# raviraj988/3D-POINT-CLOUD-SEGMENTATION-USING-2D-IMG-SEGMENTATION

Measured on AMD Instinct MI355X. Metric: labelled points/sec (10M pts x 64 views) at 1/2/4/8 GPU; % HBM roofline, higher is better.
Workload: dtype f64; 1 GPU; C3: 10000000 points x 64 ring views, 1024x1024 block64 uint8 masks, nclasses=133, threshold=0.5, filter_classes=None; fused project->sample->vote->segment; points_total=10000000, points_per_gpu=10000000, views=64, xyz_storage=f64, cloud_layout=caller order, cell-sorted inside every step (F3D_FUSE_SORT), exchange=none

## Files before the change

### 3d-point-cloud-segmentation-using-2d-img-segmentation_amd/csrc/f3d_fuse.hip

```cpp
#include <hip/hip_runtime.h>
#include <stdint.h>
#include <stdlib.h>
#include <string.h>
#include "f3d.h"
#include "f3d_math.h"
#include "f3d_kernels.h"
#include <cstdlib>

#pragma clang fp contract(off)

#define F3D_NO_PREFILL ((int64_t)0x7fffffffffffffffLL)
#define F3D_PART_MAX_GROUPS 16
#ifndef F3D_MID_DENSE
#define F3D_MID_DENSE 8
#endif
#ifndef F3D_NT_CLASSES
#define F3D_NT_CLASSES 1
#endif
#if defined(F3D_EXP_STORE) && F3D_EXP_STORE == 2
#define F3D_STORE_CLASS(p, v) ((void)(v))
#elif defined(F3D_EXP_STORE) && F3D_EXP_STORE == 3
#define F3D_STORE_CLASS(p, v) (reinterpret_cast<uint8_t*>(classes)[(p) - classes] = (uint8_t)(v))
#elif defined(F3D_EXP_STORE) && F3D_EXP_STORE == 4
#define F3D_STORE_CLASS(p, v) __builtin_nontemporal_store((uint8_t)(v), reinterpret_cast<uint8_t*>(classes) + ((p) - classes))
// ... 320 lines not shown
    bool bad = false;
};

template <int MODE>
__device__ __forceinline__ void vote_add(vote_state<MODE>& st, uint32_t* hist, int tid, const f3d_filter_args& flt, int nclasses,
                                         bool valid, int label) {
    using HT = hist_traits<MODE>;
    st.bad = st.bad | (valid & (label > nclasses));
    valid = valid & (label <= nclasses);
    st.total += valid ? 1 : 0;
    const unsigned l = valid ? (unsigned)label : (unsigned)nclasses + 1u;
    const unsigned sh = (l & (HT::per_word - 1)) * HT::bits;
    const uint32_t old = atomicAdd(&hist[(l >> HT::shift) * F3D_BLOCK + tid], 1u << sh);
    const unsigned c = ((old >> sh) & HT::mask) + 1u;
    const unsigned key = valid ? ((c << 16) | (0xFFFFu - l)) : 0u;
    st.best = st.best > key ? st.best : key;
}

template <typename FilterAt>
__device__ __forceinline__ int64_t segment_point(int win_c, int win_i, int total, int nfilter, FilterAt fat, int nclasses, double threshold,
                                                 const uint16_t* cmin = nullptr) {
    int64_t cls;
    if (total == 0) cls = nclasses;
    else {
        cls = win_i;
        const bool low = cmin ? win_c < (int)cmin[total] : (double)win_c / (double)total < threshold;
        if (low) cls = nclasses;
        if (win_c == 0) cls = nclasses;
    }
    if (nfilter > 0) {
        int64_t r = cls;
        for (int k = 0; k < nfilter; ++k) if (r == k) r = fat(k);
        cls = r;
    }
    return cls;
}

template <int MODE, bool WRITE_VOTES>
__device__ __forceinline__ void finish_point(const vote_state<MODE>& st, const uint32_t* hist, int tid, const f3d_filter_args& flt,
                                             int nclasses, double threshold, bool store, int64_t orig,
                                             int64_t* __restrict__ classes, uint16_t* __restrict__ votes_out) {
    using HT = hist_traits<MODE>;
    const int ncols = nclasses + 1;
    int win_c, win_i;
    if (flt.nfilter > 0) {
        win_c = -1; win_i = 0;
        for (int k = 0; k < flt.nfilter; ++k) {
            const int l = f3d_filter_at(flt, k);
            int c = 0;
            if (l >= 0 && l < ncols) c = (int)((hist[(l >> HT::shift) * F3D_BLOCK + tid] >> ((l & (HT::per_word - 1)) * HT::bits)) & HT::mask);
            if (c > win_c) { win_c = c; win_i = k; }
        }
    } else {
        win_c = (int)(st.best >> 16); win_i = (int)(0xFFFFu - (st.best & 0xFFFFu));
    }
    const int64_t cls = segment_point(win_c, win_i, st.total, flt.nfilter, [&](int k) { return f3d_filter_at(flt, k); }, nclasses, threshold);
    if (store) F3D_STORE_CLASS(&classes[orig], cls);
    if (WRITE_VOTES && store) {
        for (int l = 0; l < ncols; ++l)
            votes_out[(size_t)orig * ncols + l] =
                (uint16_t)((hist[(l >> HT::shift) * F3D_BLOCK + tid] >> ((l & (HT::per_word - 1)) * HT::bits)) & HT::mask);
    }
}

__device__ __forceinline__ void vote_bin32(uint32_t* hcol, unsigned b) { atomicAdd(&hcol[b * F3D_BLOCK], 1u); }

template <bool WRITE_VOTES>
__device__ __forceinline__ void finish_bin32(const uint32_t* hcol, int ncodes, const uint8_t* lut, const uint8_t* inv, int nfilter,
                                             const int* __restrict__ fcls, int nclasses, double threshold, bool store, int orig,
                                             int64_t* __restrict__ classes, uint16_t* __restrict__ votes_out, bool& bad,
                                             const uint16_t* cmin = nullptr, int64_t prefilled = F3D_NO_PREFILL) {
    const int ncols = nclasses + 1;
    const unsigned cbad = hcol[F3D_BLOCK];
    bad = cbad != 0u;
    unsigned best = 0, sum = cbad;
    for (int c = 2; c < ncodes; ++c) {
        const unsigned n = hcol[c * F3D_BLOCK];
        const unsigned key = (n << 8) | (unsigned)c;
        sum += n;
        best = best > key ? best : key;
    }
    int win_c, win_i;
    if (nfilter > 0) {
        win_c = -1; win_i = 0;
        for (int k = 0; k < nfilter; ++k) {
            const int l = fcls[k];
            int c = 0;
            if (l >= 0 && l < ncols) { const unsigned b = lut[l]; c = b >= 2u ? (int)hcol[b * F3D_BLOCK] : 0; }
            if (c > win_c) { win_c = c; win_i = k; }
        }
    } else {
        win_c = (int)(best >> 8); win_i = (int)inv[best & 0xFFu];
    }
    const int64_t cls = segment_point(win_c, win_i, (int)sum, nfilter, [&](int k) { return fcls[k]; }, nclasses, threshold, cmin);
    if (store && cls != prefilled) F3D_STORE_CLASS(&classes[orig], cls);
    if (WRITE_VOTES && store) {
        for (int l = 0; l < ncols; ++l) { const unsigned b = lut[l]; votes_out[(size_t)orig * ncols + l] = (uint16_t)(b >= 2u ? hcol[b * F3D_BLOCK] : 0u); }
    }
}

template <bool GUARD>
__device__ __forceinline__ void vote_coded(unsigned& nvalid, uint32_t* hcol, unsigned b) {
    if (GUARD) {
        const unsigned one = b < 1u ? b : 1u;
        nvalid += one;
        atomicAdd(&hcol[(b >> 2) * F3D_BLOCK], one << ((b & 3u) * 8u));
    } else {
        atomicAdd(&hcol[(b >> 2) * F3D_BLOCK], 1u << ((b & 3u) * 8u));
    }
}

__device__ __forceinline__ unsigned coded_count(const uint32_t* hcol, unsigned b) {
    return (hcol[(b >> 2) * F3D_BLOCK] >> ((b & 3u) * 8u)) & 0xFFu;
}

template <bool WRITE_VOTES, bool WRAP>
__device__ __forceinline__ bool finish_coded(unsigned nvalid, const uint32_t* hcol, int words, const uint8_t* lut, const uint8_t* inv,
                                             int nfilter, const int* __restrict__ fcls, int nclasses, double threshold, bool store,
                                             int orig, int64_t* __restrict__ classes, uint16_t* __restrict__ votes_out, bool& bad,
                                             const uint16_t* cmin = nullptr, int64_t prefilled = F3D_NO_PREFILL) {
    const int ncols = nclasses + 1;
    unsigned best = 0, sum = 0;
    {
        const unsigned x = hcol[0];
        bad = ((x >> 8) & 0xFFu) != 0u;
        const unsigned c2 = (x >> 16) & 0xFFu, c3 = x >> 24;
        sum = ((x >> 8) & 0xFFu) + c2 + c3;
        best = (c2 << 8) | 2u;
        const unsigned k3 = (c3 << 8) | 3u;
        best = best > k3 ? best : k3;
    }
    typedef unsigned short u16x2 __attribute__((ext_vector_type(2)));
    u16x2 me = {0, 0}, mo = {0, 0};
    for (int w = 1; w < words; ++w) {
        const unsigned x = hcol[w * F3D_BLOCK];
        const unsigned tag = (unsigned)w * 0x00010001u;
        sum = __builtin_amdgcn_sad_u8(x, 0u, sum);
        const unsigned o = (x & 0xFF00FF00u) | tag, e = ((x << 8) & 0xFF00FF00u) | tag;
        mo = __builtin_elementwise_max(mo, __builtin_bit_cast(u16x2, o));
        me = __builtin_elementwise_max(me, __builtin_bit_cast(u16x2, e));
    }
    {
        const unsigned cand[4] = {me.x, mo.x, me.y, mo.y};
#pragma unroll
        for (unsigned j = 0; j < 4; ++j) {
            const unsigned key = (cand[j] & 0xFF00u) | ((cand[j] & 0x3Fu) << 2) | j;
            best = best > key ? best : key;
        }
    }
    if (WRAP && sum != nvalid) return false;
    int win_c, win_i;
    if (nfilter > 0) {
        win_c = -1; win_i = 0;
        for (int k = 0; k < nfilter; ++k) {
            const int l = fcls[k];
            int c = 0;
            if (l >= 0 && l < ncols) { const unsigned b = lut[l]; c = b >= 2u ? (int)coded_count(hcol, b) : 0; }
            if (c > win_c) { win_c = c; win_i = k; }
        }
    } else {
        win_c = (int)(best >> 8); win_i = (int)inv[best & 0xFFu];
    }
    const int64_t cls = segment_point(win_c, win_i, (int)sum, nfilter, [&](int k) { return fcls[k]; }, nclasses, threshold, cmin);
    if (store && cls != prefilled) F3D_STORE_CLASS(&classes[orig], cls);
    if (WRITE_VOTES && store) {
        for (int l = 0; l < ncols; ++l) { const unsigned b = lut[l]; votes_out[(size_t)orig * ncols + l] = (uint16_t)(b >= 2u ? coded_count(hcol, b) : 0u); }
    }
    return true;
}

template <bool MAX>
__device__ __forceinline__ float wave_reduce(float v) {
#define F3D_DPP_CHAIN(op)                                                                  \
    asm volatile("s_nop 1\n\t" op " %0, %0, %0 quad_perm:[1,0,3,2] row_mask:0xf bank_mask:0xf\n\t" \
                 "s_nop 1\n\t" op " %0, %0, %0 quad_perm:[2,3,0,1] row_mask:0xf bank_mask:0xf\n\t" \
                 "s_nop 1\n\t" op " %0, %0, %0 row_half_mirror row_mask:0xf bank_mask:0xf\n\t"     \
                 "s_nop 1\n\t" op " %0, %0, %0 row_mirror row_mask:0xf bank_mask:0xf\n\t"          \
                 "s_nop 1\n\t" op " %0, %0, %0 row_bcast:15 row_mask:0xa bank_mask:0xf\n\t"        \
                 "s_nop 1\n\t" op " %0, %0, %0 row_bcast:31 row_mask:0xc bank_mask:0xf\n\t"        \
                 "s_nop 1" : "+v"(v))
    if (MAX) F3D_DPP_CHAIN("v_max_f32_dpp"); else F3D_DPP_CHAIN("v_min_f32_dpp");
#undef F3D_DPP_CHAIN
    return __int_as_float(__builtin_amdgcn_readlane(__float_as_int(v), 63));
}

__device__ __forceinline__ void wave_box(float& lo0, float& hi0, float& lo1, float& hi1, float& lo2, float& hi2) {
#define F3D_STEP(ctrl)                                                \
    "v_min_f32_dpp %0, %0, %0 " ctrl "\n\tv_max_f32_dpp %1, %1, %1 " ctrl "\n\t" \
    "v_min_f32_dpp %2, %2, %2 " ctrl "\n\tv_max_f32_dpp %3, %3, %3 " ctrl "\n\t" \
    "v_min_f32_dpp %4, %4, %4 " ctrl "\n\tv_max_f32_dpp %5, %5, %5 " ctrl "\n\t"
    asm volatile("s_nop 1\n\t"
                 F3D_STEP("quad_perm:[1,0,3,2] row_mask:0xf bank_mask:0xf")
                 F3D_STEP("quad_perm:[2,3,0,1] row_mask:0xf bank_mask:0xf")
                 F3D_STEP("row_half_mirror row_mask:0xf bank_mask:0xf")
                 F3D_STEP("row_mirror row_mask:0xf bank_mask:0xf")
                 F3D_STEP("row_bcast:15 row_mask:0xa bank_mask:0xf")
                 F3D_STEP("row_bcast:31 row_mask:0xc bank_mask:0xf")
                 "s_nop 1"
                 : "+v"(lo0), "+v"(hi0), "+v"(lo1), "+v"(hi1), "+v"(lo2), "+v"(hi2));
#undef F3D_STEP
#define F3D_L63(x) x = __int_as_float(__builtin_amdgcn_readlane(__float_as_int(x), 63))
    F3D_L63(lo0); F3D_L63(hi0); F3D_L63(lo1); F3D_L63(hi1); F3D_L63(lo2); F3D_L63(hi2);
#undef F3D_L63
}

#ifndef F3D_VTAB_GLOBAL
#define F3D_VTAB_GLOBAL 0
#endif
#ifndef F3D_XCD_CHUNK_LOG2
#define F3D_XCD_CHUNK_LOG2 6
#endif
#ifndef F3D_FUSE_WAVES
#define F3D_FUSE_WAVES 3
#endif
__device__ __forceinline__ void threshold_table(f3d_codebook* __restrict__ cb, double threshold);
__global__ __launch_bounds__(F3D_BLOCK) void k_fuse_setup(const f3d_view* __restrict__ views, int nviews, float* __restrict__ ctabT,
                                                           double* __restrict__ vtabT, f3d_codebook* __restrict__ cb, double threshold,
                                                           unsigned int* __restrict__ todo_count, int lut_nclasses, int lut_book, f3d_filter_args flt) {
    if (lut_book >= 0 && blockIdx.x == gridDim.x - 1) { code_lut_block(cb, lut_nclasses, lut_book, flt); return; }
    if (blockIdx.x == 0) {
        threshold_table(cb, threshold);
        if (todo_count && threadIdx.x < 4) todo_count[threadIdx.x] = 0u;
    }
    const int ngroups = (nviews + 63) >> 6;
    const int nsetup = lut_book >= 0 ? (int)gridDim.x - 1 : (int)gridDim.x;
    for (int k = blockIdx.x * F3D_BLOCK + threadIdx.x; k < ngroups * 64 * 39; k += nsetup * F3D_BLOCK) {
        const int v = k / 39, f = k - v * 39, g = v >> 6, l = v & 63;
        const f3d_view& vw = views[v < nviews ? v : nviews - 1];
        if (f < 24) ctabT[(g * 24 + f) * 64 + l] = reinterpret_cast<const float*>(&vw.cull_n32[0][0])[f];
        else vtabT[(g * F3D_VHEAD + (f - 24)) * 64 + l] = reinterpret_cast<const double*>(&vw)[f - 24];
    }
}

template <typename T, int PPL, bool WRITE_VOTES, bool BIN32, bool WRAP, bool TLDS, bool CARRY>
__global__ __launch_bounds__(F3D_BLOCK, F3D_FUSE_WAVES) void k_fuse(const T* __restrict__ xyz, int64_t n,
                                                     const f3d_view* __restrict__ views, int nviews,
                                                     const uint8_t* __restrict__ cmasks, int H, int W,
                                                     int nclasses, int nfilter, const int* __restrict__ fcls, double threshold,
                                                     int64_t* __restrict__ classes, uint16_t* __restrict__ votes_out,
                                                     int* __restrict__ err, const int32_t* __restrict__ perm, int gather_xyz,
                                                     unsigned int* __restrict__ todo_count, int32_t* __restrict__ todo,
                                                     const f3d_codebook* __restrict__ cb, int cmin, int cmax,
                                                     const float* __restrict__ ctabT, const double* __restrict__ vtabT,
                                                     uint32_t* __restrict__ carry, int chunk_flags, T* __restrict__ xyz_keep,
                                                     unsigned long long* __restrict__ umask, uint32_t* __restrict__ park, int park_slots, int park_stride,
                                                     int64_t prefilled) {
    const int ncodes = cb->ncodes;
    if (ncodes > cmax || ncodes < cmin) return;
    const int words = (ncodes + 3) >> 2;
    const int hdw = BIN32 ? ncodes : words;
    extern __shared__ uint32_t lds_u32[];
    float* ctab = reinterpret_cast<float*>(lds_u32);
    uint32_t* lutw = TLDS ? lds_u32 + 64 * F3D_CULL_ROW : lds_u32;
    double* vtab = reinterpret_cast<double*>(lutw + F3D_BOOK_DWORDS);
    uint32_t* hist = (TLDS && !F3D_VTAB_GLOBAL) ? lutw + F3D_BOOK_DWORDS + 2 * F3D_VHEAD * 64 : lutw + F3D_BOOK_DWORDS;
    const uint16_t* vmin = (WRAP || nviews > 255) ? nullptr : reinterpret_cast<const uint16_t*>(lutw + 128);
    const uint8_t* lut = reinterpret_cast<const uint8_t*>(lutw);
    const uint8_t* inv = lut + 256;
    const int tid = threadIdx.x, lane = threadIdx.x & 63;
    constexpr int TILE = F3D_BLOCK * PPL;
    const int npts = (int)n;
    const int ntiles = (int)((n + TILE - 1) / TILE);
    const unsigned plane = (unsigned)f3d_coded_plane(H, W);
    const int pitch = f3d_coded_pitch(W);
    const int c_row = 64 * pitch - 64;
    const int ngroups = (nviews + 63) >> 6;
    const float umaxf = (float)(W > H ? W : H), Wf = (float)W, Hf = (float)H;

    const __amdgpu_buffer_rsrc_t cm_rsrc = __builtin_amdgcn_make_buffer_rsrc(const_cast<uint8_t*>(cmasks), 0, (int)((unsigned)nviews * plane), 0x00020000);
#if defined(F3D_EXP_GATHER) && F3D_EXP_GATHER == 1
    auto gather = [&](unsigned off) -> unsigned { return (unsigned)__builtin_amdgcn_raw_buffer_load_b8(cm_rsrc, (int)(off & 63u), 0, 0); };
#elif defined(F3D_EXP_GATHER) && F3D_EXP_GATHER == 2
    auto gather = [&](unsigned off) -> unsigned { return off & 2u; };
#else
    auto gather = [&](unsigned off) -> unsigned { return (unsigned)__builtin_amdgcn_raw_buffer_load_b8(cm_rsrc, (int)off, 0, 0); };
#endif
    lutw[tid] = reinterpret_cast<const uint32_t*>(cb->lut)[tid];
    auto stage_group = [&](int g) {
        const int nv = min(64, nviews - 64 * g);
        for (int k = tid; k < nv * 24; k += F3D_BLOCK) {
            const int vi = k / 24, f = k - vi * 24;
            ctab[vi * F3D_CULL_ROW + f] = reinterpret_cast<const float*>(&views[64 * g + vi].cull_n32[0][0])[f];
        }
        if (!F3D_VTAB_GLOBAL)
            for (int k = tid; k < nv * F3D_VHEAD; k += F3D_BLOCK) {
                const int vi = k / F3D_VHEAD, f = k - vi * F3D_VHEAD;
                vtab[f * 64 + vi] = reinterpret_cast<const double*>(&views[64 * g + vi])[f];
            }
    };
    if (TLDS && ngroups > 1) return;
    if (TLDS) stage_group(0);
    __syncthreads();

    int xlog = F3D_XCD_CHUNK_LOG2;
#ifndef F3D_XCD_MIN_ROWS
#define F3D_XCD_MIN_ROWS 8
#endif
    while (xlog > 0 && ntiles < ((8 * F3D_XCD_MIN_ROWS) << xlog)) --xlog;
    const int chunk_rows = (ntiles + (8 << xlog) - 1) >> (xlog + 3);
    const int tiles_per_xcd = chunk_rows << xlog;
    const int xcd = blockIdx.x & 7, bx = blockIdx.x >> 3, gx = gridDim.x >> 3;
    uint32_t* const hcol0 = hist + tid;
    uint32_t* const hcol1 = PPL == 2 ? hist + hdw * F3D_BLOCK + tid : hcol0;
    for (int j = bx; j < tiles_per_xcd; j += gx) {
        const int tile = ((j >> xlog) << (xlog + 3)) + (xcd << xlog) + (j & ((1 << xlog) - 1));
        if (tile >= ntiles) continue;
        const int i0 = tile * TILE + (tid >> 6) * (64 * PPL) + lane;
        bool live[2], act[2], defer[2];
        int orig[2];
        f32x2 DX, DY, DZ;
        float c0, c1, c2, e0, e1, e2, ps_box;
        bool wave_any;
        {
            f3d_p3 p[2];
            float lo0 = INFINITY, lo1 = INFINITY, lo2 = INFINITY, hi0 = -INFINITY, hi1 = -INFINITY, hi2 = -INFINITY;
#pragma unroll
            for (int q = 0; q < 2; ++q) {
                const int i = i0 + 64 * q;
                live[q] = (q < PPL) & (i < npts);
                orig[q] = live[q] ? (perm ? perm[i] : i) : i;
                p[q].x = p[q].y = p[q].z = 0.0;
                if (live[q]) p[q] = f3d_load_p3(xyz, (int64_t)(gather_xyz ? orig[q] : i));
                if (CARRY && xyz_keep && live[q]) { xyz_keep[3 * (size_t)i] = (T)p[q].x; xyz_keep[3 * (size_t)i + 1] = (T)p[q].y; xyz_keep[3 * (size_t)i + 2] = (T)p[q].z; }
                const double pscale = (fabs(p[q].x) + fabs(p[q].y)) + fabs(p[q].z);
                act[q] = live[q] & (pscale < 1.0e30);
                defer[q] = live[q] & !act[q];
                const float x32 = (float)p[q].x, y32 = (float)p[q].y, z32 = (float)p[q].z;
                if (act[q]) {
                    lo0 = fminf(lo0, x32); hi0 = fmaxf(hi0, x32); lo1 = fminf(lo1, y32); hi1 = fmaxf(hi1, y32);
                    lo2 = fminf(lo2, z32); hi2 = fmaxf(hi2, z32);
                }
            }
            wave_box(lo0, hi0, lo1, hi1, lo2, hi2);
            wave_any = __any(act[0] | act[1]);
            c0 = 0.5f * (lo0 + hi0); c1 = 0.5f * (lo1 + hi1); c2 = 0.5f * (lo2 + hi2);
            e0 = 0.5f * (hi0 - lo0) * 1.000002f + 1e-30f; e1 = 0.5f * (hi1 - lo1) * 1.000002f + 1e-30f;
            e2 = 0.5f * (hi2 - lo2) * 1.000002f + 1e-30f;
            ps_box = ((fabsf(c0) + fabsf(c1)) + fabsf(c2)) + ((e0 + e1) + e2);
            DX = (f32x2){(float)(p[0].x - (double)c0), (float)(p[1].x - (double)c0)};
            DY = (f32x2){(float)(p[0].y - (double)c1), (float)(p[1].y - (double)c1)};
            DZ = (f32x2){(float)(p[0].z - (double)c2), (float)(p[1].z - (double)c2)};
            if (!act[0]) { DX.x = __builtin_nanf(""); }
            if (!act[1]) { DX.y = __builtin_nanf(""); }
        }
        constexpr bool PART = !CARRY;
        const bool part_rt = PART && park_slots > 0 && ngroups <= F3D_PART_MAX_GROUPS;
        unsigned long long um[2] = {0ull, 0ull};
        int slot[2] = {-1, -1};
        unsigned unsure[2] = {0u, 0u};
        if (CARRY && (chunk_flags & 1)) {
#pragma unroll
            for (int q = 0; q < PPL; ++q) {
                uint32_t* hc = q ? hcol1 : hcol0;
                const uint32_t* cq = carry + ((size_t)(tile * PPL + q) * words) * F3D_BLOCK + tid;
                for (int wd = 0; wd < words; ++wd) {
                    uint32_t x = cq[wd * F3D_BLOCK];
                    if (wd == 0) { defer[q] = defer[q] | (live[q] & ((x & 0xFFu) != 0u)); x &= ~0xFFu; }
                    if (BIN32) {
#pragma unroll
                        for (int b4 = 0; b4 < 4; ++b4) if (4 * wd + b4 < ncodes) hc[(4 * wd + b4) * F3D_BLOCK] = (x >> (8 * b4)) & 0xFFu;
                    } else {
                        hc[wd * F3D_BLOCK] = x;
                    }
                }
            }
        } else {
            for (int wd = 0; wd < hdw; ++wd) { hcol0[wd * F3D_BLOCK] = 0u; if (PPL == 2) hcol1[wd * F3D_BLOCK] = 0u; }
        }
        unsigned nvalid[2] = {0u, 0u};
        unsigned pend[2] = {F3D_CODE_NONE, F3D_CODE_NONE};
        unsigned ccode[2][F3D_CHUNK];
#pragma unroll
        for (int k = 0; k < F3D_CHUNK; ++k) ccode[0][k] = ccode[1][k] = F3D_CODE_NONE;
#if F3D_GATHER_DEPTH == 2
        unsigned ccode2[2][F3D_CHUNK];
#pragma unroll
        for (int k = 0; k < F3D_CHUNK; ++k) ccode2[0][k] = ccode2[1][k] = F3D_CODE_NONE;
#define F3D_OLDEST ccode2
#else
#define F3D_OLDEST ccode
#endif
        auto vote = [&](int q, unsigned b) {
            if (q >= PPL) return;
            if (BIN32) vote_bin32(q ? hcol1 : hcol0, b);
            else vote_coded<WRAP || CARRY>(nvalid[q], q ? hcol1 : hcol0, b);
        };

        for (int g = 0; g < ngroups; ++g) {
            const int vj = 64 * g + lane;
            bool box_out = false, box_in = true, own_image = false;
            float pb0 = 0.f, pb1 = 0.f, pb2 = 0.f, pb3 = 0.f, pb4 = 0.f, pmarg = 0.f;
            unsigned pneed = 0u;
            if (vj < nviews) {
                const float* rowp = TLDS ? ctab + lane * F3D_CULL_ROW : ctabT + (size_t)g * 24 * 64 + lane;
                auto rowf = [&](int f) { return TLDS ? rowp[f] : rowp[f * 64]; };
                const float marg = 2.0f * __builtin_fmaf(rowf(20), ps_box, rowf(21));
                float bmax = 0.f, smax = 0.f, base[F3D_NPLANES];
                unsigned need = 0u;
#pragma unroll
                for (int m = 0; m < F3D_NPLANES; ++m) {
                    const float n0 = rowf(3 * m), n1 = rowf(3 * m + 1), n2 = rowf(3 * m + 2);
                    base[m] = __builtin_fmaf(n0, c0, __builtin_fmaf(n1, c1, __builtin_fmaf(n2, c2, -rowf(15 + m))));
                    const float spread = __builtin_fmaf(fabsf(n0), e0, __builtin_fmaf(fabsf(n1), e1, fabsf(n2) * e2));
                    box_out = box_out | (base[m] + spread < -marg);
                    box_in = box_in & (base[m] - spread > marg);
                    need |= (base[m] - spread > marg) ? 0u : (1u << m);
                    bmax = fmaxf(bmax, fabsf(base[m])); smax = fmaxf(smax, spread);
                }
                pb0 = base[0]; pb1 = base[1]; pb2 = base[2]; pb3 = base[3]; pb4 = base[4];
                pneed = need;
                pmarg = 0.5f * marg + 1.01f * (float)F3D_U24 * (4.0f * bmax + 5.0f * smax);
                own_image = (int)(rowf(22) == Wf) & (int)(rowf(23) == Hf);
            }
            centre_row mine = {0.f, 0.f, 0.f, 0.f, 0.f, 0.f, 0.f, 0.f, 0.f, 0.f, 0.f, 0.f, 0u, 0, 0};
            bool row_ok = false;
            if (vj < nviews && !box_out && wave_any)
                row_ok = centre_precompute((TLDS && !F3D_VTAB_GLOBAL) ? vtab + lane : vtabT + (size_t)g * F3D_VHEAD * 64 + lane, 64, c0, c1, c2, e0, e1, e2, umaxf, pitch, mine);
            mine.obase += (unsigned)vj * plane;
            const unsigned long long valid_m = __ballot(vj < nviews);
            unsigned long long out_m = __ballot(vj < nviews && box_out);
            const unsigned long long in_m = __ballot(vj < nviews && box_in && !box_out && own_image);
            const unsigned long long row_m = __ballot(row_ok);
            if (!wave_any) out_m = valid_m;
            unsigned long long todo_v = valid_m & ~out_m & in_m & row_m;
#if defined(F3D_EXP_SKIP) && (F3D_EXP_SKIP == 1 || F3D_EXP_SKIP == 3)
            todo_v = 0ull;
#endif
            while (todo_v) {
                int cbit[F3D_CHUNK]; unsigned coff[2][F3D_CHUNK];
                bool use[F3D_CHUNK];
                unsigned long long unsm[2][F3D_CHUNK];
#pragma unroll
                for (int k = 0; k < F3D_CHUNK; ++k) {
                    use[k] = todo_v != 0ull;
                    cbit[k] = use[k] ? __builtin_ctzll(todo_v) : (k ? cbit[0] : 0);
                    if (use[k]) todo_v &= todo_v - 1ull;
                }
#pragma unroll
                for (int k = 0; k < F3D_CHUNK; ++k) {
                    const centre_row r = read_row(mine, cbit[k]);
                    int fi0[2], fi1[2]; bool safe[2];
                    project_offset2(r, DX, DY, DZ, fi0, fi1, safe);
#pragma unroll
                    for (int q = 0; q < PPL; ++q) {
                        if (PART) unsm[q][k] = __ballot(act[q] & !safe[q]);
                        else unsure[q] = safe[q] ? unsure[q] : 1u;
                        const unsigned o = r.obase + rel_offset(fi0[q], fi1[q], c_row);
                        coff[q][k] = (safe[q] & use[k]) ? o : 0u;
                    }
                }
#ifndef F3D_NO_VOTE_PIN
#pragma unroll
                for (int k = 0; k < F3D_CHUNK; ++k) {
                    asm volatile("" : "+v"(F3D_OLDEST[0][k]) : "v"(coff[0][k]));
                    if (PPL == 2) asm volatile("" : "+v"(F3D_OLDEST[1][k]) : "v"(coff[1][k]));
                }
#endif
#pragma unroll
                for (int k = 0; k < F3D_CHUNK; ++k) { vote(0, F3D_OLDEST[0][k]); vote(1, F3D_OLDEST[1][k]); }
#if F3D_GATHER_DEPTH == 2
#pragma unroll
                for (int k = 0; k < F3D_CHUNK; ++k) { ccode2[0][k] = ccode[0][k]; ccode2[1][k] = ccode[1][k]; }
#endif
#pragma unroll
                for (int k = 0; k < F3D_CHUNK; ++k) { ccode[0][k] = gather(coff[0][k]); if (PPL == 2) ccode[1][k] = gather(coff[1][k]); }
                if (PART) {
                    unsigned long long au = 0ull;
#pragma unroll
                    for (int k = 0; k < F3D_CHUNK; ++k) au |= unsm[0][k] | (PPL == 2 ? unsm[1][k] : 0ull);
                    if (__builtin_expect(au != 0ull, 0)) {
                        asm volatile("" ::: "memory");
                        const unsigned long long me = 1ull << lane;
#pragma unroll
                        for (int k = 0; k < F3D_CHUNK; ++k)
#pragma unroll
                            for (int q = 0; q < PPL; ++q) um[q] |= (unsm[q][k] & me) ? (1ull << cbit[k]) : 0ull;
                    }
                }
            }
#pragma unroll
            for (int k = 0; k < F3D_CHUNK; ++k) {
#if F3D_GATHER_DEPTH == 2
                vote(0, ccode2[0][k]); vote(1, ccode2[1][k]);
                ccode2[0][k] = ccode2[1][k] = F3D_CODE_NONE;
#endif
                vote(0, ccode[0][k]); vote(1, ccode[1][k]);
                ccode[0][k] = ccode[1][k] = F3D_CODE_NONE;
            }
            todo_v = valid_m & ~out_m & ~(in_m & row_m);
#if defined(F3D_EXP_SKIP) && F3D_EXP_SKIP == 2
            todo_v = 0ull;
#elif defined(F3D_EXP_SKIP) && F3D_EXP_SKIP == 3
            todo_v = 0ull;
#endif
            while (todo_v) {
                const int bit = __builtin_ctzll(todo_v);
                todo_v &= todo_v - 1ull;
                const int v = 64 * g + bit;
                const f3d_view& vw = views[v];
                float nn[F3D_NPLANES][3];
#pragma unroll
                for (int m = 0; m < F3D_NPLANES; ++m) { nn[m][0] = vw.cull_n32[m][0]; nn[m][1] = vw.cull_n32[m][1]; nn[m][2] = vw.cull_n32[m][2]; }
#pragma unroll
                for (int m = 0; m < F3D_NPLANES; ++m) { asm volatile("" : "+s"(nn[m][0])); asm volatile("" : "+s"(nn[m][1])); asm volatile("" : "+s"(nn[m][2])); }
#define F3D_RL1(x) __int_as_float(__builtin_amdgcn_readlane(__float_as_int(x), bit))
                const float mg = F3D_RL1(pmarg);
                const unsigned need = (unsigned)__builtin_amdgcn_readlane((int)pneed, bit);
                const float* pbs[F3D_NPLANES] = {&pb0, &pb1, &pb2, &pb3, &pb4};
                const bool has_row = (row_m >> bit) & 1ull;
                bool maybe[2] = {true, true}, sure[2] = {true, true};
#pragma unroll
                for (int m = 0; m < F3D_NPLANES; ++m) {
                    if (!((need >> m) & 1u)) continue;
                    const float bbm = F3D_RL1(*pbs[m]);
                    const f32x2 a = F3D_FMA2(splat2(nn[m][0]), DX, F3D_FMA2(splat2(nn[m][1]), DY, F3D_FMA2(splat2(nn[m][2]), DZ, splat2(bbm))));
                    maybe[0] = maybe[0] & (a.x > -mg); sure[0] = sure[0] & (a.x > mg);
                    maybe[1] = maybe[1] & (a.y > -mg); sure[1] = sure[1] & (a.y > mg);
                }
#undef F3D_RL1
                unsigned off[2] = {0u, 0u};
                bool unsv[2] = {false, false};
                if (has_row) {
                    centre_row r = read_row(mine, bit);
                    const int U8 = __builtin_amdgcn_readlane(mine.U8, bit), V8 = __builtin_amdgcn_readlane(mine.V8, bit);
                    int fi0[2], fi1[2]; bool safe[2];
                    project_offset2(r, DX, DY, DZ, fi0, fi1, safe);
#pragma unroll
                    for (int q = 0; q < PPL; ++q) {
                        const bool inside = sure[q];
                        const bool hit = inside & safe[q] & ((unsigned)(fi0[q] + U8) < (unsigned)W) & ((unsigned)(fi1[q] + V8) < (unsigned)H);
                        unsv[q] = (maybe[q] & !sure[q]) | (inside & !safe[q]);
                        const unsigned o = r.obase + rel_offset(fi0[q], fi1[q], c_row);
                        off[q] = hit ? o : 0u;
                    }
                } else {
#pragma unroll
                    for (int q = 0; q < PPL; ++q) unsv[q] = maybe[q];
                }
                if (PART) {
                    const unsigned long long u0 = __ballot(unsv[0] & act[0]), u1 = __ballot(unsv[1] & act[1]);
                    if (__builtin_expect((u0 | u1) != 0ull, 0)) {
                        asm volatile("" ::: "memory");
                        const unsigned long long me = 1ull << lane;
                        um[0] |= (u0 & me) ? (1ull << bit) : 0ull;
                        if (PPL == 2) um[1] |= (u1 & me) ? (1ull << bit) : 0ull;
                    }
                } else {
#pragma unroll
                    for (int q = 0; q < PPL; ++q) unsure[q] = unsv[q] ? 1u : unsure[q];
                }
#ifndef F3D_NO_VOTE_PIN
                asm volatile("" : "+v"(pend[0]) : "v"(off[0]));
                if (PPL == 2) asm volatile("" : "+v"(pend[1]) : "v"(off[1]));
#endif
                vote(0, pend[0]); vote(1, pend[1]);
                pend[0] = gather(off[0]); if (PPL == 2) pend[1] = gather(off[1]);
            }
            if (PART && __any(((um[0] | um[1]) != 0ull) | (slot[0] >= 0) | (slot[1] >= 0))) {
#pragma unroll
                for (int q = 0; q < PPL; ++q) {
                    if (!part_rt) { unsure[q] = um[q] != 0ull ? 1u : unsure[q]; }
                    else if (act[q] && (um[q] != 0ull || slot[q] >= 0)) {
                        if (slot[q] < 0) {
                            slot[q] = (int)atomicAdd(todo_count, 1u);
                            if (slot[q] < park_slots) for (int gg = 0; gg < g; ++gg) umask[(size_t)slot[q] * ngroups + gg] = 0ull;
                        }
                        if (slot[q] < park_slots) umask[(size_t)slot[q] * ngroups + g] = um[q];
                    }
                    um[q] = 0ull;
                }
            }
        }
#pragma unroll
        for (int q = 0; q < PPL; ++q) {
            vote(q, pend[q]);
            const bool part = act[q] & ((PART && slot[q] >= 0) | (unsure[q] != 0u));
            bool full = defer[q] | (part & !part_rt);
            defer[q] = defer[q] | part;
            uint32_t* hc = q ? hcol1 : hcol0;
            if (CARRY && (chunk_flags & 2)) {
                uint32_t* cq = carry + ((size_t)(tile * PPL + q) * words) * F3D_BLOCK + tid;
                for (int wd = 0; wd < words; ++wd) {
                    uint32_t x = 0u;
                    if (BIN32) {
#pragma unroll
                        for (int b4 = 0; b4 < 4; ++b4) if (4 * wd + b4 < ncodes) x |= (hc[(4 * wd + b4) * F3D_BLOCK] & 0xFFu) << (8 * b4);
                    } else {
                        x = hc[wd * F3D_BLOCK];
                    }
                    if (wd == 0) x = (x & ~0xFFu) | (defer[q] ? 1u : 0u);
                    cq[wd * F3D_BLOCK] = x;
                }
                continue;
            }
            bool bad = false, trusted = true;
            if (BIN32) finish_bin32<WRITE_VOTES>(hc, ncodes, lut, inv, nfilter, fcls, nclasses, threshold, live[q] & !defer[q], orig[q], classes, votes_out, bad, vmin, prefilled);
            else trusted = finish_coded<WRITE_VOTES, WRAP>(nvalid[q], hc, words, lut, inv, nfilter, fcls, nclasses, threshold, live[q] & !defer[q], orig[q],
                                                           classes, votes_out, bad, vmin, prefilled);
            full = full | (live[q] & !trusted);
            const bool d = defer[q] | full;
            if (d) {
                const int sl = (PART && slot[q] >= 0) ? slot[q] : (int)atomicAdd(todo_count, 1u);
                full = full | !part_rt | (sl >= park_slots) | !(PART && slot[q] >= 0);
                if (BIN32 && !full && nviews > 255)
                    for (int c = 1; c < ncodes; ++c) full = full | (hc[c * F3D_BLOCK] > 255u);
                todo[sl] = (gather_xyz ? orig[q] : (i0 + 64 * q)) | (full ? (int)0x80000000 : 0);
                if (PART && !full) {
                    uint32_t* pk = park + (size_t)sl * park_stride;
                    for (int wd = 0; wd < words; ++wd) {
                        uint32_t x = 0u;
                        if (BIN32) {
#pragma unroll
                            for (int b4 = 0; b4 < 4; ++b4) if (4 * wd + b4 < ncodes) x |= (hc[(4 * wd + b4) * F3D_BLOCK] & 0xFFu) << (8 * b4);
                        } else {
                            x = hc[wd * F3D_BLOCK];
                        }
                        pk[wd] = wd == 0 ? (x & ~0xFFu) : x;
                    }
                }
            }
            if (bad & !d) atomicOr(err, F3D_DEVERR_FUSE);
        }
    }
}

__device__ __forceinline__ void cull_point64(const f3d_view& vw, f3d_p3 p, double pscale, bool& maybe, bool& sure) {
    const double marg = __builtin_fma(vw.cull_rel64, pscale, vw.cull_abs64);
    bool mb = true, sr = true;
#pragma unroll
    for (int m = 0; m < F3D_NPLANES; ++m) {
        const double a = __builtin_fma(vw.plane_n[m][0], p.x, __builtin_fma(vw.plane_n[m][1], p.y,
                         __builtin_fma(vw.plane_n[m][2], p.z, -vw.plane_off[m])));
        mb = mb & (a > -marg);
        sr = sr & (a > marg);
    }
    maybe = mb; sure = sr;
}

__device__ __forceinline__ bool project_fast(const f3d_view& vw, double umax, f3d_p3 p, int W, int H, int& iu, int& iv, bool& unsure) {
    const double d0 = p.x - vw.t[0], d1 = p.y - vw.t[1], d2 = p.z - vw.t[2];
    const double h0 = __builtin_fma(vw.M[0], d0, __builtin_fma(vw.M[1], d1, vw.M[2] * d2));
    const double h1 = __builtin_fma(vw.M[3], d0, __builtin_fma(vw.M[4], d1, vw.M[5] * d2));
    const double h2 = __builtin_fma(vw.M[6], d0, __builtin_fma(vw.M[7], d1, vw.M[8] * d2));
    const double r = rcp_newton(h2);
    const double uf = h0 * r, vf = h1 * r;
    const double fu = floor(uf), fv = floor(vf);
    const double c1 = __builtin_fma(umax, vw.mnorm[2], fmax(vw.mnorm[0], vw.mnorm[1]));
    const double b = F3D_FAST_EPS * __builtin_fma(((fabs(d0) + fabs(d1)) + fabs(d2)) * fabs(r), c1, umax);
    const bool safe = (fabs((uf - fu) - 0.5) < 0.5 - b) && (fabs((vf - fv) - 0.5) < 0.5 - b);
    unsure = !safe;
    iu = (int)fu; iv = (int)fv;
    return safe & ((unsigned)iu < (unsigned)W) & ((unsigned)iv < (unsigned)H);
}

template <typename T, bool WRITE_VOTES>
__global__ __launch_bounds__(F3D_BLOCK) void k_fuse_mid(const T* __restrict__ xyz, const unsigned int* __restrict__ in_count, const int32_t* __restrict__ in_list,
                                                         const f3d_view* __restrict__ views, int nviews,
                                                         const uint8_t* __restrict__ cmasks, int H, int W,
                                                         int nclasses, int nfilter, const int* __restrict__ fcls, double threshold,
                                                         int64_t* __restrict__ classes, uint16_t* __restrict__ votes_out,
                                                         int* __restrict__ err, const int32_t* __restrict__ perm, int gather_xyz,
                                                         unsigned int* __restrict__ out_count, int32_t* __restrict__ out_list,
                                                         unsigned int* __restrict__ diag_count, const f3d_codebook* __restrict__ cb,
                                                         const unsigned long long* __restrict__ umask, const uint32_t* __restrict__ park,
                                                         int park_slots, int park_stride) {
    extern __shared__ uint32_t lds_u32[];
    uint32_t* lutw = lds_u32;
    uint32_t* spre = lutw + 128;
    uint32_t* snv = spre + F3D_BLOCK + 4;
    uint32_t* sdefer = snv + F3D_BLOCK;
    unsigned long long* smask = reinterpret_cast<unsigned long long*>(sdefer + F3D_BLOCK);
    double* spt = reinterpret_cast<double*>(smask + F3D_BLOCK);
    uint32_t* hist = reinterpret_cast<uint32_t*>(spt + 3 * F3D_BLOCK);
    const uint8_t* lut = reinterpret_cast<const uint8_t*>(lutw);
    const uint8_t* inv = lut + 256;
    const int tid = threadIdx.x, lane = tid & 63, wv = tid >> 6;
    const int words = cb->words;
    const size_t plane = f3d_coded_plane(H, W);
    const int wt = f3d_coded_pitch(W);
    const unsigned none_off = 0u;
    const double umax = (double)(W > H ? W : H);
    const int ngroups = (nviews + 63) >> 6;
    if (tid < 128) lutw[tid] = reinterpret_cast<const uint32_t*>(cb->lut)[tid];
    const int count = (int)*in_count;
    for (int base = blockIdx.x * F3D_BLOCK; base < count; base += gridDim.x * F3D_BLOCK) {
        const int k = base + tid;
        const bool live = k < count;
        const int entry = live ? in_list[k] : 0;
        const int src = entry & 0x7fffffff;
        const bool full = (entry < 0) | (k >= park_slots) | (umask == nullptr);
        {
            f3d_p3 p = {0.0, 0.0, 0.0};
            if (live) p = f3d_load_p3(xyz, (int64_t)src);
            spt[tid] = p.x; spt[F3D_BLOCK + tid] = p.y; spt[2 * F3D_BLOCK + tid] = p.z;
            sdefer[tid] = 0u;
            unsigned nv0 = 0;
            if (live && !full) {
                const uint32_t* pk = park + (size_t)k * park_stride;
                for (int wd = 0; wd < words; ++wd) {
                    const uint32_t x = pk[wd];
                    hist[wd * F3D_BLOCK + tid] = x;
                    nv0 = __builtin_amdgcn_sad_u8(x, 0u, nv0);
                }
            } else {
                for (int wd = 0; wd < words; ++wd) hist[wd * F3D_BLOCK + tid] = 0u;
            }
            snv[tid] = nv0;
        }
        for (int g = 0; g < ngroups; ++g) {
            const int nvg = min(64, nviews - 64 * g);
            unsigned long long m = !live ? 0ull : full ? (nvg == 64 ? ~0ull : (1ull << nvg) - 1ull) : umask[(size_t)k * ngroups + g];
#if defined(F3D_EXP_MID) && F3D_EXP_MID == 1
            m = 0ull;
#elif defined(F3D_EXP_MID) && F3D_EXP_MID == 2
            m &= 0ull - m;
#endif
            const unsigned c = (unsigned)__builtin_popcountll(m);
            unsigned incl = c;
#pragma unroll
            for (int off = 1; off < 64; off <<= 1) { const unsigned o = __shfl_up(incl, off, 64); incl += lane >= off ? o : 0u; }
            __syncthreads();
            smask[tid] = m;
            if (lane == 63) spre[F3D_BLOCK + wv] = incl;
            __syncthreads();
            unsigned wbase = 0, total = 0;
#pragma unroll
            for (int w = 0; w < F3D_BLOCK / 64; ++w) { const unsigned t = spre[F3D_BLOCK + w]; wbase += w < wv ? t : 0u; total += t; }
            spre[tid] = wbase + incl - c;
            __syncthreads();
            unsigned pend_code = F3D_CODE_NONE;
            int pend_pt = 0;
            auto cast = [&](int pt, unsigned b) {
                if (b != F3D_CODE_NONE) { atomicAdd(&snv[pt], 1u); atomicAdd(&hist[(b >> 2) * F3D_BLOCK + pt], 1u << ((b & 3u) * 8u)); }
            };
            auto pair = [&](int pt, const f3d_p3& p, int v, const f3d_view& vw, bool on) {
                bool hit = false;
                int iu = 0, iv = 0;
                const double pscale = (fabs(p.x) + fabs(p.y)) + fabs(p.z);
                const bool small = on & (pscale < 1.0e30);
                bool exact = on & !small;
                bool maybe, sure;
                cull_point32(load_cull(vw), (float)p.x, (float)p.y, (float)p.z, (float)pscale, small, maybe, sure);
                bool inside = small & sure;
                if (small & maybe & !sure) {
                    bool m64, s64;
                    cull_point64(vw, p, pscale, m64, s64);
                    inside = s64;
                    exact = exact | (m64 & !s64);
                }
                if (inside) {
                    bool unsure;
                    hit = project_fast(vw, umax, p, W, H, iu, iv, unsure);
                    exact = exact | unsure;
                }
                if (exact) {
                    hit = false;
                    if (f3d_inside_view(vw, p)) {
                        double fu, fv;
                        project_exact(vw, p, fu, fv);
                        if (fu >= 0.0 && fu < (double)W && fv >= 0.0 && fv < (double)H) { hit = true; iu = (int)fu; iv = (int)fv; }
                    }
                    atomicOr(&sdefer[pt], 1u);
                }
                cast(pend_pt, pend_code);
                pend_code = (cmasks + (size_t)v * plane)[hit ? mask_offset<true>(iu, iv, wt) : none_off];
                pend_pt = pt;
            };
            if (total > (unsigned)F3D_BLOCK * F3D_MID_DENSE) {
                const f3d_p3 p = {spt[tid], spt[F3D_BLOCK + tid], spt[2 * F3D_BLOCK + tid]};
                for (int bit = 0; bit < nvg; ++bit) {
                    const bool on = (m >> bit) & 1ull;
                    if (!__any(on)) continue;
                    pair(tid, p, 64 * g + bit, views[64 * g + bit], on);
                }
            } else {
                for (unsigned j = tid; j < total; j += F3D_BLOCK) {
                    int lo = 0;
#pragma unroll
                    for (int step = F3D_BLOCK / 2; step >= 1; step >>= 1) lo += (spre[lo + step] <= j) ? step : 0;
                    unsigned long long mm = smask[lo];
                    for (unsigned r = j - spre[lo]; r > 0; --r) mm &= mm - 1ull;
                    const int v = 64 * g + __builtin_ctzll(mm);
                    const f3d_p3 p = {spt[lo], spt[F3D_BLOCK + lo], spt[2 * F3D_BLOCK + lo]};
                    pair(lo, p, v, views[v], true);
                }
            }
            cast(pend_pt, pend_code);
        }
        __syncthreads();
        const int orig = (live && perm && !gather_xyz) ? perm[src] : src;
        bool bad = false;
        const bool trusted = finish_coded<WRITE_VOTES, true>(snv[tid], hist + tid, words, lut, inv, nfilter, fcls, nclasses, threshold,
                                                             live, orig, classes, votes_out, bad);
        const bool defer = live & !trusted;
        if (defer && out_list) out_list[atomicAdd(out_count, 1u)] = src;
        if (live && diag_count && sdefer[tid] != 0u) atomicAdd(diag_count, 1u);
        if (bad & !defer) atomicOr(err, F3D_DEVERR_FUSE);
        __syncthreads();
    }
}

template <typename T, int MODE, bool WRITE_VOTES>
__global__ __launch_bounds__(F3D_BLOCK) void k_fuse_exact(const T* __restrict__ xyz, int64_t n_all, const unsigned int* __restrict__ todo_count,
                                                           const int32_t* __restrict__ todo,
                                                           const f3d_view* __restrict__ views, int nviews,
                                                           const uint8_t* __restrict__ masks, int H, int W,
                                                           int nclasses, f3d_filter_args flt, double threshold,
                                                           int64_t* __restrict__ classes, uint16_t* __restrict__ votes_out,
                                                           int* __restrict__ err, const int32_t* __restrict__ perm,
                                                           int gather_xyz) {
    using HT = hist_traits<MODE>;
    extern __shared__ uint32_t lds_u32[];
    uint32_t* hist = lds_u32;
    const int tid = threadIdx.x;
    const int ncols = nclasses + 1;
    const int words = (ncols + 1 + HT::per_word - 1) >> HT::shift;
    const size_t plane = (size_t)H * (size_t)W;
    const int64_t count = todo ? (int64_t)*todo_count : n_all;
    for (int64_t base = (int64_t)blockIdx.x * F3D_BLOCK; base < count; base += (int64_t)gridDim.x * F3D_BLOCK) {
        const int64_t k = base + tid;
        const bool live = k < count;
        const int64_t src = live ? (todo ? (int64_t)todo[k] : k) : 0;
        const int64_t orig = (live && perm && !gather_xyz) ? (int64_t)perm[src] : src;
        f3d_p3 p = {0.0, 0.0, 0.0};
        if (live) p = f3d_load_p3(xyz, src);
        for (int wd = 0; wd < words; ++wd) hist[wd * F3D_BLOCK + tid] = 0u;
        vote_state<MODE> st;
        for (int v = 0; v < nviews; ++v) {
            const f3d_view& vw = views[v];
            bool hit = false;
            unsigned off = 0u;
            if (live && f3d_inside_view(vw, p)) {
                double fu, fv;
                project_exact(vw, p, fu, fv);
                if (fu >= 0.0 && fu < (double)W && fv >= 0.0 && fv < (double)H) {
                    hit = true; off = mask_offset<false>((int)fu, (int)fv, W);
                }
            }
            const int label = hit ? (int)(masks + (size_t)v * plane)[off] : 0;
            vote_add<MODE>(st, hist, tid, flt, nclasses, hit, label);
        }
        if (st.bad) atomicOr(err, F3D_DEVERR_FUSE);
        finish_point<MODE, WRITE_VOTES>(st, hist, tid, flt, nclasses, threshold, live, orig, classes, votes_out);
    }
}

template <typename T>
__global__ __launch_bounds__(F3D_BLOCK) void k_fastpath_audit(const T* __restrict__ xyz, int64_t n,
                                                               const f3d_view* __restrict__ views, int nviews, int W, int H,
                                                               unsigned long long* __restrict__ stats) {
    unsigned long long pairs = 0, fallback = 0, wrong = 0, cullwrong = 0;
    const int lane = threadIdx.x & 63;
    const int64_t ntiles = (n + F3D_BLOCK - 1) / F3D_BLOCK;
    const float umaxf = (float)(W > H ? W : H);
    for (int64_t tile = blockIdx.x; tile < ntiles; tile += gridDim.x) {
        const int64_t i = tile * F3D_BLOCK + threadIdx.x;
        const bool live = i < n;
        f3d_p3 p = {0.0, 0.0, 0.0};
        if (live) p = f3d_load_p3(xyz, i);
        const double pscale = (fabs(p.x) + fabs(p.y)) + fabs(p.z);
        const bool small = pscale < 1.0e30;
        const float px32 = (float)p.x, py32 = (float)p.y, pz32 = (float)p.z;
        float lo0 = INFINITY, lo1 = INFINITY, lo2 = INFINITY, hi0 = -INFINITY, hi1 = -INFINITY, hi2 = -INFINITY;
        if (live & small) { lo0 = hi0 = px32; lo1 = hi1 = py32; lo2 = hi2 = pz32; }
        lo0 = wave_reduce<false>(lo0); hi0 = wave_reduce<true>(hi0);
        lo1 = wave_reduce<false>(lo1); hi1 = wave_reduce<true>(hi1);
        lo2 = wave_reduce<false>(lo2); hi2 = wave_reduce<true>(hi2);
        const bool wave_any = __any(live & small);
        const float c0 = 0.5f * (lo0 + hi0), c1 = 0.5f * (lo1 + hi1), c2 = 0.5f * (lo2 + hi2);
        const float e0 = 0.5f * (hi0 - lo0) * 1.000002f + 1e-30f, e1 = 0.5f * (hi1 - lo1) * 1.000002f + 1e-30f,
                    e2 = 0.5f * (hi2 - lo2) * 1.000002f + 1e-30f;
        const float ps_box = ((fabsf(c0) + fabsf(c1)) + fabsf(c2)) + ((e0 + e1) + e2);
        const float dx32 = (float)(p.x - (double)c0), dy32 = (float)(p.y - (double)c1), dz32 = (float)(p.z - (double)c2);
        for (int g = 0; g < (nviews + 63) / 64; ++g) {
            const int vj = 64 * g + lane;
// ... 301 lines not shown
```

Before: 10.91 billion points/s.

## Add optional software prefetch of next tile's perm and point coordinates

Restructures the tile loop so the permutation index and xyz coordinates for the next tile can be loaded early, while the current tile's view loop runs, hiding global load latency. Placement is selected by F3D_PF_PLACE; the default (0) issues the loads at the top of the current tile, which matches the original ordering but goes through the new helper lambdas and register staging. With prefetch enabled, registers stay live across the whole view loop, which may lower occupancy.

```diff
diff --git a/3d-point-cloud-segmentation-using-2d-img-segmentation_amd/csrc/f3d_fuse.hip b/3d-point-cloud-segmentation-using-2d-img-segmentation_amd/csrc/f3d_fuse.hip
--- a/3d-point-cloud-segmentation-using-2d-img-segmentation_amd/csrc/f3d_fuse.hip
+++ b/3d-point-cloud-segmentation-using-2d-img-segmentation_amd/csrc/f3d_fuse.hip
@@ -646,10 +646,46 @@
     const int xcd = blockIdx.x & 7, bx = blockIdx.x >> 3, gx = gridDim.x >> 3;
     uint32_t* const hcol0 = hist + tid;
     uint32_t* const hcol1 = PPL == 2 ? hist + hdw * F3D_BLOCK + tid : hcol0;
-    for (int j = bx; j < tiles_per_xcd; j += gx) {
-        const int tile = ((j >> xlog) << (xlog + 3)) + (xcd << xlog) + (j & ((1 << xlog) - 1));
-        if (tile >= ntiles) continue;
-        const int i0 = tile * TILE + (tid >> 6) * (64 * PPL) + lane;
+#ifndef F3D_PF_PLACE
+#define F3D_PF_PLACE 0
+#endif
+    auto tile_at = [&](int j) { return ((j >> xlog) << (xlog + 3)) + (xcd << xlog) + (j & ((1 << xlog) - 1)); };
+    auto next_pos = [&](int j) {
+        while (j < tiles_per_xcd && tile_at(j) >= ntiles) j += gx;
+        return j;
+    };
+    auto lane_i0 = [&](int j) { return j < tiles_per_xcd ? tile_at(j) * TILE + (tid >> 6) * (64 * PPL) + lane : npts; };
+    int nxt_orig[2] = {0, 0};
+    T nxt_p[2][3] = {{(T)0, (T)0, (T)0}, {(T)0, (T)0, (T)0}};
+    auto request_perm = [&](int i0n) {
+#pragma unroll
+        for (int q = 0; q < PPL; ++q) {
+            const int i = i0n + 64 * q;
+            nxt_orig[q] = (i < npts && perm) ? perm[i] : i;
+        }
+    };
+    auto request_points = [&](int i0n) {
+        asm volatile("" :: "v"(nxt_orig[0]));
+        if (PPL == 2) asm volatile("" :: "v"(nxt_orig[1]));
+#pragma unroll
+        for (int q = 0; q < PPL; ++q) {
+            const int i = i0n + 64 * q;
+#ifdef F3D_EXP_NOPERM
+            const T* src = xyz + 3 * (int64_t)i;
+#else
+            const T* src = xyz + 3 * (int64_t)(gather_xyz ? nxt_orig[q] : i);
+#endif
+            nxt_p[q][0] = nxt_p[q][1] = nxt_p[q][2] = (T)0;
+            if (i < npts) { nxt_p[q][0] = src[0]; nxt_p[q][1] = src[1]; nxt_p[q][2] = src[2]; }
+        }
+    };
+    int j = next_pos(bx);
+    if (F3D_PF_PLACE != 0) { request_perm(lane_i0(j)); request_points(lane_i0(j)); }
+    for (; j < tiles_per_xcd;) {
+        const int tile = tile_at(j);
+        const int i0 = lane_i0(j);
+        j = next_pos(j + gx);
+        const int i0_next = lane_i0(j);
         bool live[2], act[2], defer[2];
         int orig[2];
         f32x2 DX, DY, DZ;
@@ -658,13 +694,13 @@
         {
             f3d_p3 p[2];
             float lo0 = INFINITY, lo1 = INFINITY, lo2 = INFINITY, hi0 = -INFINITY, hi1 = -INFINITY, hi2 = -INFINITY;
+            if (F3D_PF_PLACE == 0) { request_perm(i0); request_points(i0); }
 #pragma unroll
             for (int q = 0; q < 2; ++q) {
                 const int i = i0 + 64 * q;
                 live[q] = (q < PPL) & (i < npts);
-                orig[q] = live[q] ? (perm ? perm[i] : i) : i;
-                p[q].x = p[q].y = p[q].z = 0.0;
-                if (live[q]) p[q] = f3d_load_p3(xyz, (int64_t)(gather_xyz ? orig[q] : i));
+                orig[q] = q < PPL ? nxt_orig[q] : i;
+                p[q].x = (double)nxt_p[q][0]; p[q].y = (double)nxt_p[q][1]; p[q].z = (double)nxt_p[q][2];
                 if (CARRY && xyz_keep && live[q]) { xyz_keep[3 * (size_t)i] = (T)p[q].x; xyz_keep[3 * (size_t)i + 1] = (T)p[q].y; xyz_keep[3 * (size_t)i + 2] = (T)p[q].z; }
                 const double pscale = (fabs(p[q].x) + fabs(p[q].y)) + fabs(p[q].z);
                 act[q] = live[q] & (pscale < 1.0e30);
@@ -687,6 +723,7 @@
             if (!act[0]) { DX.x = __builtin_nanf(""); }
             if (!act[1]) { DX.y = __builtin_nanf(""); }
         }
+        if (F3D_PF_PLACE != 0) request_perm(i0_next);
         constexpr bool PART = !CARRY;
         const bool part_rt = PART && park_slots > 0 && ngroups <= F3D_PART_MAX_GROUPS;
         unsigned long long um[2] = {0ull, 0ull};
@@ -831,6 +868,7 @@
                 vote(0, ccode[0][k]); vote(1, ccode[1][k]);
                 ccode[0][k] = ccode[1][k] = F3D_CODE_NONE;
             }
+            if (F3D_PF_PLACE == 1 && g == ngroups - 1) request_points(i0_next);
             todo_v = valid_m & ~out_m & ~(in_m & row_m);
 #if defined(F3D_EXP_SKIP) && F3D_EXP_SKIP == 2
             todo_v = 0ull;
@@ -915,6 +953,7 @@
                 }
             }
         }
+        if (F3D_PF_PLACE == 2 || (F3D_PF_PLACE == 1 && ngroups == 0)) request_points(i0_next);
 #pragma unroll
         for (int q = 0; q < PPL; ++q) {
             vote(q, pend[q]);
```

New measurement: 10.90 billion points/s. No clear change (-0.1%).
